# itz-sayak/C-Users-Sayakdutta-Self-Supervised-Arbitrary-Scale-Point-Cloud-Upsampling-via-SNN

Measured on AMD Instinct MI355X. Metric: upsampled query-points/sec (kNN + fn fwd + rotate + fd fwd + displace), 4x scale, M=48 T=4, higher is better.
Workload: dtype f32 (GEMMs as 3 x f16 MFMA with f32 accumulation; outer kNN f64); 1 GPU; synthetic sphere N=5000 (seed 0), B=4096 grid queries per GPU per step, M=48, T=4, fn k=[24,18,12] emb 640, fd k=32 scales [8,16,32,48] emb 768, conditioned-random weights seed 0, in-patch kNN recomputed every batch; cloud_points=5000, neighbours=48, outer_knn=f64 brute force, parallelism=query shards x1

## Files before the change

c-users-sayakdutta-self-supervised-arbitrary-scale-point-cloud-upsampling-via-snn_amd/csrc/common.h:

```cpp
#pragma once
#include <hip/hip_runtime.h>
#include <stdint.h>
#include <stdio.h>
#include <string.h>
#include "../../include/sapcu.h"

namespace sapcu {

void set_error(const char* fmt, ...);

#define SAPCU_CHECK_ARG(cond, ...)                      \
    do {                                                \
        if (!(cond)) {                                  \
            ::sapcu::set_error(__VA_ARGS__);            \
            return SAPCU_ERR_ARG;                       \
        }                                               \
    } while (0)

#define SAPCU_CHECK_HIP(expr)                                                            \
    do {                                                                                 \
        hipError_t _e = (expr);                                                          \
        if (_e != hipSuccess) {                                                          \
            ::sapcu::set_error("%s failed: %s (%s:%d)", #expr, hipGetErrorString(_e),    \
                               __FILE__, __LINE__);                                      \
// ... 343 lines not shown
    }
    __device__ __forceinline__ bool gate_open() const {
#ifdef SAPCU_LIF_EXACT_ORDER
        return sx.r <= 0.f || sy.r <= 0.f;
#else
        return s.r.x <= 0.f || s.r.y <= 0.f;
#endif
    }
    __device__ __forceinline__ f32x2 step(f32x2 x, bool first) {
#ifdef SAPCU_LIF_EXACT_ORDER
        return f32x2{neuron_step<EIF>(x.x, sx, pa), neuron_step<EIF>(x.y, sy, pb)};
#else
        f32x2 mm;
        if (first) {
            mm = x;
        } else {
            const f32x2 md = s.m * decay;
            mm = pk_fma(-md, s.r, md);
        }
        if (EIF) {
            f32x2 a = (s.m - rh) * inv_dT;
            a = f32x2{clampf(a.x, -5.0f, 5.0f), clampf(a.y, -5.0f, 5.0f)} * 1.4426950408889634074f;
            const f32x2 e = f32x2{__builtin_amdgcn_exp2f(a.x), __builtin_amdgcn_exp2f(a.y)};
            mm = pk_fma(e, dT, mm);
        }
        const f32x2 sp = soft_spike2(mm - s.th);
        s.m = pk_fma(-mm, sp, mm);
        {
            const f32x2 rn = first ? sp : pk_fma(s.r, rdecay, sp);
            s.r = f32x2{fmaxf(rn.x, SPIKE_FLOOR), fmaxf(rn.y, SPIKE_FLOOR)};
        }
        s.th = pk_fma(s.th, f32x2{0.95f, 0.95f}, pk_fma(sp, a95, thc));
        return sp;
#endif
    }
};

__device__ __forceinline__ double sqrt_cr(double d) {
    if (!(d > 0.0)) return d == 0.0 ? 0.0 : sqrt(d);
    const double s = sqrt(d);
    const double r = __fma_rn(-s, s, d);
    return __fma_rn(r, __ddiv_rn(0.5, s), s);
}

__device__ __forceinline__ float gelu_erf(float x) {
    return 0.5f * x * (1.0f + erff(x * 0.70710678118654752440f));
}
__device__ __forceinline__ float lrelu02(float x) { return x >= 0.f ? x : 0.2f * x; }
__device__ __forceinline__ unsigned float_max_key(float x) {
    const unsigned b = __float_as_uint(x);
    return (b & 0x80000000u) ? ~b : (b | 0x80000000u);
}
__device__ __forceinline__ float float_from_max_key(unsigned k) { return __uint_as_float((k & 0x80000000u) ? (k & 0x7fffffffu) : ~k); }

enum GemmEpi { EPI_BIAS = 0, EPI_LIF = 1, EPI_GELU = 2, EPI_RESID = 3, EPI_LRELU = 4, EPI_RESID_GELU = 5, EPI_LIF_ATTN = 6,
               EPI_LRELU_MAX = 7,
               EPI_LIF_MAX = 8 };

struct GemmArgs {
    const float* a;
    int64_t r;
    int k, lda;
    const float* w;
    int n;
    const float* bias;
    float* c;
    int ldc;
    int epi;
    const float* lif;
    int lif_T;
    const float* resid;
    int ldr;
    float* c2;
    const float* q;
    const float* kf;
    int ldq;
    const int2* tab;
    const _Float16* w16_hi;
    const _Float16* w16_lo;
    int* ovf;
    int a_split, c_split, c2_split;
    unsigned* max_keys;
    int max_m;
};
int launch_gemm(const GemmArgs& g, hipStream_t st);
int launch_gemm_sf16(const GemmArgs& g, hipStream_t st);
int launch_gemm_sf16_ring(const GemmArgs& g, hipStream_t st);
int launch_gemm_sf16_bt(const GemmArgs& g, hipStream_t st);
bool gemm_sf16_bt_ok(const GemmArgs& g);
int launch_gemm_split_rows(const GemmArgs& g, hipStream_t st, bool allow_bt = true);
int launch_split_weights(const float* w, int64_t count, void* hi, void* lo, int* ovf, hipStream_t st);

int launch_knn_outer(const double* cloud, int64_t n, const double* q, int64_t b, int k, int64_t* idx,
                     double* dist, float* patch, hipStream_t st);
int launch_gather_rotate(const double* cloud, int64_t n, const double* q, int64_t b, const int64_t* idx,
                         int k, const float* normals, float* patch, hipStream_t st);
int launch_displace(const double* q, const float* nrm, const float* d, int64_t b, double* out, hipStream_t st);

size_t fps_workspace_bytes(int npoint);
int launch_fps(const float* xyz, int64_t n, int npoint, int start, int64_t* out, void* ws, hipStream_t st);
int fps_failed(const void* ws, int npoint, int* flag);

}
```

c-users-sayakdutta-self-supervised-arbitrary-scale-point-cloud-upsampling-via-snn_amd/csrc/model.hip:

```cpp
#include <stdarg.h>
#include <stdlib.h>

#include <new>
#include <vector>

#include "common.h"
#include "ops.h"

namespace sapcu {

static thread_local char g_err[512] = "";

void set_error(const char* fmt, ...) {
    va_list ap;
    va_start(ap, fmt);
    vsnprintf(g_err, sizeof(g_err), fmt, ap);
    va_end(ap);
}

enum FnSlot {
    FN_STEM_W = 0, FN_STEM_B, FN_STEM_LIF,
    FN_BLK0 = 3,
    FN_FINAL_W = FN_BLK0 + 63, FN_FINAL_B, FN_FINAL_LIF,
    FN_FCOUT_W, FN_FCOUT_B,
    FN_MLP0_W, FN_MLP0_B, FN_MLP1_W, FN_MLP1_B, FN_MLP2_W, FN_MLP2_B,
    FN_HEAD_W, FN_HEAD_B, FN_LN_W, FN_LN_B,
    FN_SLOTS
};
enum FnBlkSlot {
    B_FC1_W = 0, B_FC1_B, B_SNN1,
    B_QKV_W, B_QKV_B, B_QKV_LIF,
    B_DELTA_W, B_DELTA_B, B_DELTA_LIF,
    B_DELTA2_W, B_DELTA2_B, B_DELTA2_LIF,
    B_GAMMA_W, B_GAMMA_B, B_GAMMA_LIF,
    B_GAMMA2_W, B_GAMMA2_B,
    B_OUT_W, B_OUT_B,
    B_FC2_W, B_FC2_B,
    B_SLOTS
};
static_assert(B_SLOTS == 21, "fn block slot count");
static_assert(FN_SLOTS == 81, "fn slot count");

enum FdSlot {
    FD_E0_W = 0, FD_E0_B,
    FD_FUSE_W, FD_FUSE_B, FD_SNN0,
    FD_EDGE1_W, FD_EDGE1_SHIFT, FD_SNN1,
    FD_EDGE2_W, FD_EDGE2_SHIFT, FD_SNN2,
    FD_EDGE3_W, FD_EDGE3_SHIFT, FD_SNN3,
    FD_MSC_W, FD_MSC_B,
    FD_TI_W, FD_SNNFC,
    FD_FCIN_W, FD_FCIN_B,
    FD_R0_FC0_W, FD_R0_FC0_B, FD_R0_FC4_W, FD_R0_FC4_B, FD_R0_PROJ_W, FD_R0_PROJ_B,
    FD_R1_FC0_W, FD_R1_FC0_B, FD_R1_FC4_W, FD_R1_FC4_B, FD_R1_PROJ_W, FD_R1_PROJ_B,
    FD_QKV_W, FD_QKV_B,
    FD_WO_T, FD_BO, FD_LN_W, FD_LN_B, FD_WH_T, FD_BH, FD_WD, FD_BD,
    FD_SLOTS
};
static_assert(FD_SLOTS == 42, "fd slot count");

}

struct sapcu_model {
    int kind = 0;
    int kv[3] = {0, 0, 0};
    int k = 0, nscale = 0;
    int ks[8] = {0, 0, 0, 0, 0, 0, 0, 0};
    int32_t* ks_dev = nullptr;
    int* gate_dev = nullptr;
    bool sf16 = true;
    void* w16_hi = nullptr;
    void* w16_lo = nullptr;
    void* chain_w = nullptr;
    int* ovf_dev = nullptr;
    int emb = 0, T = 0, heads = 0;
    int64_t chunk = 0;
    int64_t ws_budget = 0;
    bool opt_bt = true;
    bool opt_chain = true;
    bool opt_chain_wide = false;
    bool opt_chain_fill = true;
    bool opt_fn_maxfuse = true;
    bool opt_fn_fold_out = true;
    bool opt_fd_maxfuse = true;
    bool opt_fd_split = true;
    bool opt_fd_fused = true;
    bool opt_fd_x0 = true;
    void* fde_w = nullptr;
    int64_t fde_off[5] = {0, 0, 0, 0, 0};
    float* fde_nprm = nullptr;
    float* blob = nullptr;
    int64_t blob_floats = 0;
    int64_t fold_w[3] = {0, 0, 0}, fold_b[3] = {0, 0, 0};
    std::vector<int64_t> dir;
    const float* p(int slot) const { return blob + dir[slot]; }
};

namespace sapcu {

static inline int64_t imax(int64_t a, int64_t b) { return a > b ? a : b; }
static inline int imin(int a, int b) { return a < b ? a : b; }

static bool split_rows_gemm_on_big_tile(const GemmArgs& g, bool allow_bt) { return allow_bt && gemm_sf16_bt_ok(g); }

int launch_gemm_split_rows(const GemmArgs& g, hipStream_t st, bool allow_bt) {
    if (split_rows_gemm_on_big_tile(g, allow_bt)) return launch_gemm_sf16_bt(g, st);
    return launch_gemm_sf16_ring(g, st);
}

static void fold_affine_f64(const float* w1, const float* b1, const float* w2, const float* b2, int d, int n, float* w_fold,
                            float* b_fold) {
    std::vector<double> acc((size_t)d);
    for (int i = 0; i < n; ++i) {
        for (int k = 0; k < d; ++k) acc[k] = 0.0;
        double bs = 0.0;
        for (int j = 0; j < d; ++j) {
            const double a = (double)w2[(int64_t)i * d + j];
            const float* row = w1 + (int64_t)j * d;
            for (int k = 0; k < d; ++k) acc[k] += a * (double)row[k];
            bs += a * (double)b1[j];
        }
        for (int k = 0; k < d; ++k) w_fold[(int64_t)i * d + k] = (float)acc[k];
        b_fold[i] = (float)(bs + (double)b2[i]);
    }
}

static bool env_is(const char* name, const char* value) {
    const char* e = getenv(name);
    return e && strcmp(e, value) == 0;
}

static void read_env_switches(sapcu_model* m) {
    m->sf16 = !env_is("SAPCU_GEMM", "f32");
    m->opt_bt = !env_is("SAPCU_BT", "0");
    m->opt_chain = !env_is("SAPCU_CHAIN", "0");
    m->opt_chain_wide = env_is("SAPCU_CHAIN", "wide");
    m->opt_chain_fill = !env_is("SAPCU_CHAIN_FILL", "0");
    m->opt_fn_maxfuse = !env_is("SAPCU_FN_MAXFUSE", "0");
    m->opt_fn_fold_out = !env_is("SAPCU_FN_FOLD_OUT", "0");
    m->opt_fd_maxfuse = !env_is("SAPCU_FD_MAXFUSE", "0");
    m->opt_fd_split = !env_is("SAPCU_FD_SPLIT", "0");
    m->opt_fd_fused = !env_is("SAPCU_FD_FUSED", "0");
    m->opt_fd_x0 = !env_is("SAPCU_FD_X0", "0");
    const char* ce = getenv("SAPCU_CHUNK");
    m->chunk = ce ? atoll(ce) : 0;
    if (m->chunk < 0) m->chunk = 0;
    const char* be = getenv("SAPCU_WS_BUDGET_MB");
    m->ws_budget = (be ? atoll(be) : 20480) * (int64_t)(1 << 20);
    if (m->ws_budget < (int64_t)(64 << 20)) m->ws_budget = (int64_t)(64 << 20);
}

static void free_model(sapcu_model* m) {
    void* const owned[] = {m->w16_hi, m->w16_lo, m->chain_w, m->ovf_dev, m->blob, m->ks_dev, m->gate_dev, m->fde_w, m->fde_nprm};
    for (void* p : owned)
        if (p) (void)hipFree(p);
    delete m;
}

static int run_gemm(const sapcu_model* m, GemmArgs& g, hipStream_t st) {
    const bool have16 = m && m->sf16 && g.w >= m->blob && g.w < m->blob + m->blob_floats;
    if (have16) {
        const int64_t off = g.w - m->blob;
        g.w16_hi = (const _Float16*)m->w16_hi + off;
        g.w16_lo = (const _Float16*)m->w16_lo + off;
        g.ovf = m->ovf_dev;
        if (g.a_split) return launch_gemm_split_rows(g, st, m->opt_bt);
        if (g.k % 64 == 0) return launch_gemm_sf16(g, st);
    }
    if (g.a_split || g.c_split || g.c2_split) {
        set_error("run_gemm: split-row operands need the split-f16 kernels");
        return SAPCU_ERR_ARG;
    }
    return launch_gemm(g, st);
}

static int gemm(const sapcu_model* m, const float* a, int64_t r, int k, int lda, const float* w, int n,
                const float* bias, float* c, int ldc, int epi, hipStream_t st, const float* lif = nullptr,
                int lifT = 0, const float* resid = nullptr, int ldr = 0, int fmt = 0) {
    GemmArgs g;
    memset(&g, 0, sizeof(g));
    g.a = a; g.r = r; g.k = k; g.lda = lda; g.w = w; g.n = n; g.bias = bias; g.c = c; g.ldc = ldc;
    g.epi = epi; g.lif = lif; g.lif_T = lifT; g.resid = resid; g.ldr = ldr;
    g.a_split = fmt & 1; g.c_split = (fmt >> 1) & 1;
    return run_gemm(m, g, st);
}

#define SAPCU_TRY(expr)                 \
    do {                                \
        int _rc = (expr);               \
        if (_rc != SAPCU_OK) return _rc; \
    } while (0)

static int tap_copy(void* const* taps, int which, int64_t dst_off_bytes, const void* src, int64_t bytes,
                    hipStream_t st) {
    if (!taps || !taps[which] || bytes == 0) return SAPCU_OK;
    SAPCU_CHECK_HIP(hipMemcpyAsync((char*)taps[which] + dst_off_bytes, src, (size_t)bytes, hipMemcpyDeviceToDevice, st));
    return SAPCU_OK;
}

struct FnPlan {
    int64_t cb;
    int kk[3], kmx;
    int64_t edge_floats, edge_floats23;
};

static bool fn_block_fused(const sapcu_model* m, int l, int mp) {
    return m->sf16 && m->chain_w && m->opt_chain && fn_edge_chain_ok(128 << l, imin(m->kv[l], mp));
}

static int fn_kmax(const sapcu_model* m, int mp) {
    int kmx = 1;
    for (int l = 0; l < 3; ++l) kmx = kmx > imin(m->kv[l], mp) ? kmx : imin(m->kv[l], mp);
    return kmx;
}

static void fn_edge_floats_per_patch(const sapcu_model* m, int mp, int64_t& first, int64_t& others) {
    first = (int64_t)mp * m->emb;
    others = 0;
    for (int l = 0; l < 3; ++l) {
        if (fn_block_fused(m, l, mp)) continue;
        const int64_t e = (int64_t)mp * imin(m->kv[l], mp) * (128 << l);
        first = imax(first, e);
        others = imax(others, e);
    }
}

static int64_t fn_bytes_per_patch(const sapcu_model* m, int mp) {
    int64_t e1, e23;
    fn_edge_floats_per_patch(m, mp, e1, e23);
    int64_t idxs = 0;
    for (int l = 0; l < 3; ++l) idxs += (int64_t)mp * imin(m->kv[l], mp) * 4;
    return (e1 + 2 * e23) * 4 + idxs + (int64_t)mp * fn_kmax(m, mp) * 24 + (int64_t)mp * (64 + 192 + 512 + 1536 + 512) * 4 +
           ((int64_t)m->emb + 2048 + 1024 + 512 + 256 + 3) * 4;
}

static int64_t chunk_patches(const sapcu_model* m, int64_t b, int64_t bytes_per_patch) {
    int64_t cb = m->chunk;
    if (cb <= 0) {
        cb = m->ws_budget / (bytes_per_patch > 0 ? bytes_per_patch : 1);
        cb = cb < 64 ? 64 : (cb / 64) * 64;
    }
    if (cb > b) cb = b;
    return cb < 1 ? 1 : cb;
}

static FnPlan fn_plan(const sapcu_model* m, int64_t b, int mp) {
    FnPlan pl;
    pl.cb = chunk_patches(m, b, fn_bytes_per_patch(m, mp));
    for (int l = 0; l < 3; ++l) pl.kk[l] = imin(m->kv[l], mp);
// ... 87 lines not shown
        GemmArgs g;
        memset(&g, 0, sizeof(g));
        g.a = W.B1; g.r = R; g.k = d; g.lda = d; g.w = m->p(sb + B_DELTA2_W); g.n = d;
        g.bias = m->p(sb + B_DELTA2_B); g.c = W.B2; g.ldc = d; g.epi = EPI_LIF_ATTN;
        g.lif = m->p(sb + B_DELTA2_LIF); g.lif_T = 4; g.c2 = W.B3;
        g.q = W.QKV; g.kf = W.QKV + d; g.ldq = 3 * d; g.tab = W.tab;
        g.a_split = SP; g.c2_split = SP;
        SAPCU_TRY(launch_edge_table(idx, R, e.mp, kk, W.tab, st));
        SAPCU_TRY(run_gemm(m, g, st));
    }
    SAPCU_TRY(gemm(m, W.B3, R, d, d, m->p(sb + B_GAMMA_W), d, m->p(sb + B_GAMMA_B), W.B1, d, EPI_LIF, st, m->p(sb + B_GAMMA_LIF), 4,
                   nullptr, 0, SP | (SP << 1)));
    SAPCU_TRY(gemm(m, W.B1, R, d, d, m->p(sb + B_GAMMA2_W), d, m->p(sb + B_GAMMA2_B), W.B3, d, EPI_BIAS, st, nullptr, 0, nullptr, 0, SP));
    return launch_fn_softmax_agg(W.B3, W.B2, W.QKV + 2 * d, 3 * d, idx, e.P, e.mp, kk, d, e.sqrt_hd, W.RES, SP, st);
}

static int fn_forward(const sapcu_model* m, const float* patch, int64_t b, int mp, const int32_t* knn_in,
                      int32_t* knn_out, float* normals, void* ws, int64_t ws_bytes, void* const* taps,
                      hipStream_t st) {
    const FnPlan pl = fn_plan(m, b, mp);
    const FnWs W = fn_ws_layout(ws_align256(ws), m, pl, mp);
    if (ws_bytes < (int64_t)W.bytes + 256) {
        set_error("fn_forward: workspace %lld B < required %lld B", (long long)ws_bytes, (long long)W.bytes + 256);
        return SAPCU_ERR_WORKSPACE;
    }
    int64_t tab_off[3];
    tab_off[0] = 0;
    tab_off[1] = b * mp * pl.kk[0];
    tab_off[2] = tab_off[1] + b * mp * pl.kk[1];

    for (int64_t s = 0; s < b; s += pl.cb) {
        const int64_t cb = (b - s) < pl.cb ? (b - s) : pl.cb;
        const int64_t P = cb * mp;
        const float* pc = patch + s * mp * 3;

        if (!knn_in) SAPCU_TRY(launch_patch_knn_multi(pc, cb, (int64_t)mp * 3, mp, 3, 3, 3, pl.kk, W.idx, st));
        for (int l = 0; l < 3; ++l) {
            const int64_t cnt = P * pl.kk[l];
            if (knn_in)
                SAPCU_CHECK_HIP(hipMemcpyAsync(W.idx[l], knn_in + tab_off[l] + s * mp * pl.kk[l], cnt * 4,
                                               hipMemcpyDeviceToDevice, st));
            if (knn_out)
                SAPCU_CHECK_HIP(hipMemcpyAsync(knn_out + tab_off[l] + s * mp * pl.kk[l], W.idx[l], cnt * 4,
                                               hipMemcpyDeviceToDevice, st));
        }
        SAPCU_TRY(launch_fn_stem(pc, P, m->p(FN_STEM_W), m->p(FN_STEM_B), m->p(FN_STEM_LIF), m->T, W.feat0, st));
        SAPCU_TRY(tap_copy(taps, SAPCU_FN_TAP_STEM, s * mp * 64 * 4, W.feat0, P * 64 * 4, st));

        const float* fin = W.feat0;
        int ldin = 64;
        for (int l = 0; l < 3; ++l) {
            const int d = 128 << l;
            const int sb = FN_BLK0 + l * B_SLOTS;
            const int SP = m->sf16 ? 1 : 0;
            float* const out = W.cat + 64 * l;
            SAPCU_TRY(gemm(m, fin, P, 64, ldin, m->p(sb + B_FC1_W), d, m->p(sb + B_FC1_B), W.X, d, EPI_LIF, st,
                           m->p(sb + B_SNN1), 4, nullptr, 0, SP << 1));
            SAPCU_TRY(gemm(m, W.X, P, d, d, m->p(sb + B_QKV_W), 3 * d, m->p(sb + B_QKV_B), W.QKV, 3 * d, EPI_LIF, st,
                           m->p(sb + B_QKV_LIF), 4, nullptr, 0, SP));
            const FnEdge e{pc, P, mp, l, d, pl.kk[l], sb, SP, (float)sqrt((double)(d / m->heads)), pl.edge_floats};
            SAPCU_TRY(fn_block_fused(m, l, mp) ? fn_edge_chain_fused(m, W, e, st) : fn_edge_chain_unfused(m, W, e, st));
            if (m->opt_fn_fold_out) {
                SAPCU_TRY(gemm(m, W.RES, P, d, d, m->blob + m->fold_w[l], 64, m->blob + m->fold_b[l], out, 192, EPI_RESID, st,
                               nullptr, 0, fin, ldin, SP));
            } else {
                SAPCU_TRY(gemm(m, W.RES, P, d, d, m->p(sb + B_OUT_W), d, m->p(sb + B_OUT_B), W.X, d, EPI_BIAS, st, nullptr, 0, nullptr,
                               0, SP | (SP << 1)));
                SAPCU_TRY(gemm(m, W.X, P, d, d, m->p(sb + B_FC2_W), 64, m->p(sb + B_FC2_B), out, 192, EPI_RESID, st,
                               nullptr, 0, fin, ldin, SP));
            }
            if (taps && taps[SAPCU_FN_TAP_BLOCK1 + l]) {
                SAPCU_CHECK_HIP(hipMemcpy2DAsync((char*)taps[SAPCU_FN_TAP_BLOCK1 + l] + s * mp * 64 * 4, 64 * 4,
                                                 out, 192 * 4, 64 * 4, (size_t)P, hipMemcpyDeviceToDevice, st));
            }
            fin = out;
            ldin = 192;
        }
        if (m->sf16 && m->opt_fn_maxfuse) {
            GemmArgs g;
            memset(&g, 0, sizeof(g));
            g.a = W.cat; g.r = P; g.k = 192; g.lda = 192; g.w = m->p(FN_FINAL_W); g.n = m->emb; g.bias = m->p(FN_FINAL_B);
            g.ldc = m->emb; g.epi = EPI_LIF_MAX; g.lif = m->p(FN_FINAL_LIF); g.lif_T = m->T;
            g.max_keys = reinterpret_cast<unsigned*>(W.B1); g.max_m = mp;
            SAPCU_CHECK_HIP(hipMemsetAsync(g.max_keys, 0, (size_t)cb * m->emb * 4, st));
            SAPCU_TRY(run_gemm(m, g, st));
            SAPCU_TRY(launch_decode_max_keys(g.max_keys, cb * m->emb, W.pooled, st));
        } else {
            SAPCU_TRY(gemm(m, W.cat, P, 192, 192, m->p(FN_FINAL_W), m->emb, m->p(FN_FINAL_B), W.B1, m->emb, EPI_LIF, st,
                           m->p(FN_FINAL_LIF), m->T));
            SAPCU_TRY(launch_rowgroup_max(W.B1, cb, mp, m->emb, W.pooled, st));
        }
        SAPCU_TRY(tap_copy(taps, SAPCU_FN_TAP_POOLED, s * m->emb * 4, W.pooled, cb * m->emb * 4, st));
        SAPCU_TRY(gemm(m, W.pooled, cb, m->emb, m->emb, m->p(FN_FCOUT_W), 2048, m->p(FN_FCOUT_B), W.enc, 2048, EPI_BIAS, st));
        SAPCU_TRY(tap_copy(taps, SAPCU_FN_TAP_ENC, s * 2048 * 4, W.enc, cb * 2048 * 4, st));
        SAPCU_TRY(gemm(m, W.enc, cb, 2048, 2048, m->p(FN_MLP0_W), 1024, m->p(FN_MLP0_B), W.h1, 1024, EPI_GELU, st));
        SAPCU_TRY(gemm(m, W.h1, cb, 1024, 1024, m->p(FN_MLP1_W), 512, m->p(FN_MLP1_B), W.h2, 512, EPI_GELU, st));
        SAPCU_TRY(gemm(m, W.h2, cb, 512, 512, m->p(FN_MLP2_W), 256, m->p(FN_MLP2_B), W.h3, 256, EPI_GELU, st));
        SAPCU_TRY(launch_fn_tail(W.h3, cb, 256, m->p(FN_HEAD_W), m->p(FN_HEAD_B), m->p(FN_LN_W), m->p(FN_LN_B), W.logits,
                                 normals + s * 3, st));
        SAPCU_TRY(tap_copy(taps, SAPCU_FN_TAP_LOGITS, s * 3 * 4, W.logits, cb * 3 * 4, st));
    }
    return SAPCU_OK;
}

struct FdPlan {
    int64_t cb;
    int kmax0, kk;
    bool fused;
    bool x0path;
    bool maxfuse;
    int64_t agg_rows(int mp) const { return maxfuse ? 1 : mp; }
};

static bool fd_encoder_fused(const sapcu_model* m, int mp) {
    return m->sf16 && m->opt_fd_fused && m->fde_w && m->fde_nprm && fd_encoder_ok(mp, m->nscale, m->emb, m->T);
}

static bool fd_x0_path(const sapcu_model* m, int mp) {
    return !fd_encoder_fused(m, mp) && m->sf16 && m->opt_fd_fused && m->opt_fd_x0 && m->opt_fd_maxfuse && m->opt_fd_split && m->fde_w &&
           m->fde_nprm && fd_msc_ok(mp, m->emb, m->T);
}

static int fd_kmax0(const sapcu_model* m, int mp) {
    int kmax = 1;
    for (int i = 0; i < m->nscale; ++i) kmax = kmax > m->ks[i] ? kmax : m->ks[i];
    return imin(kmax, mp);
}

static FdPlan fd_plan(const sapcu_model* m, int64_t b, int mp) {
    FdPlan pl;
    pl.fused = fd_encoder_fused(m, mp);
    pl.x0path = fd_x0_path(m, mp);
    pl.maxfuse = m->sf16 && m->opt_fd_maxfuse;
    pl.kmax0 = fd_kmax0(m, mp);
    pl.kk = imin(m->k, mp);
    int64_t per_patch = ((int64_t)(m->T + 1) * m->emb + 256 + 3 * 128 + 3 * 64 + 192 + 64) * 4;
    if (!pl.fused) {
        const int64_t slabs = pl.x0path ? 2 : m->T;
        per_patch = (int64_t)mp * ((slabs * 960 + 960 + 1024 + 64 * (m->nscale + 1)) * 4 + (int64_t)(pl.kmax0 + 3 * pl.kk) * 4) +
                    (int64_t)m->T * pl.agg_rows(mp) * m->emb * 4 + per_patch;
    }
    pl.cb = chunk_patches(m, b, per_patch);
    return pl;
}

struct FdWs {
    int32_t* idx0;
    int32_t* idxb;
    float* E0;
    float* FUSED;
    float* SPK;
    float* F0;
    float* AB;
    float* AGG;
    float* X0;
    float *POOLED, *ENC;
    float *D1, *D2a, *D2b, *D2c, *D3a, *D3b, *D3c, *QKV, *ATT;
    size_t bytes;
};

static FdWs fd_ws_layout(void* base, const sapcu_model* m, const FdPlan& pl, int mp) {
    const int64_t cb = pl.cb, T = m->T, emb = m->emb;
    const int64_t P = pl.fused ? 0 : cb * mp;
    WsCarver c(base);
    FdWs w;
    w.idx0 = c.take<int32_t>(P * pl.kmax0);
    w.idxb = c.take<int32_t>(3 * P * pl.kk);
    w.E0 = c.take<float>(P * 64 * m->nscale);
    w.FUSED = c.take<float>(P * 64);
// ... 226 lines not shown
                    (long long)n, (long long)npoint);
    if (npoint == 0) return SAPCU_OK;
    SAPCU_CHECK_ARG(xyz && idx_out && workspace, "fps: null pointer");
    SAPCU_CHECK_ARG(((uintptr_t)workspace & 7) == 0, "fps: the workspace must be 8-byte aligned (64-bit mailboxes)");
    if (workspace_bytes < (int64_t)fps_workspace_bytes((int)npoint)) {
        set_error("fps: workspace of %lld bytes, need %lld", (long long)workspace_bytes,
                  (long long)fps_workspace_bytes((int)npoint));
        return SAPCU_ERR_WORKSPACE;
    }
    int rc = launch_fps(xyz, n, (int)npoint, (int)(n / 2), idx_out, workspace, (hipStream_t)stream);
    if (rc != SAPCU_OK) return rc;
    SAPCU_CHECK_HIP(hipStreamSynchronize((hipStream_t)stream));
    int flag = 0;
    rc = fps_failed(workspace, (int)npoint, &flag);
    if (rc != SAPCU_OK) return rc;
    if (flag) {
        set_error("fps: a workgroup of the persistent grid never arrived at the step barrier (grid not resident)");
        return SAPCU_ERR_HIP;
    }
    return SAPCU_OK;
}

int sapcu_neuron_selfloop(const float* x, int64_t rows, int channels, int steps, const float* membrane_decay,
                          const float* threshold_adapt, const float* refractory_decay, const float* threshold_base,
                          const float* delta_T, const float* theta_rh, float* spikes_out, float* membrane_out,
                          float* threshold_out, float* refractory_out, void* stream) {
    SAPCU_CHECK_ARG(x && membrane_decay && threshold_adapt && refractory_decay && threshold_base, "neuron: null pointer");
    SAPCU_CHECK_ARG((delta_T == nullptr) == (theta_rh == nullptr), "neuron: delta_T and theta_rh go together");
    SAPCU_CHECK_ARG(rows >= 0 && channels >= 1 && steps >= 1, "neuron: bad sizes");
    return launch_neuron_selfloop(x, rows, channels, steps, membrane_decay, threshold_adapt, refractory_decay,
                                  threshold_base, delta_T, theta_rh, spikes_out, membrane_out, threshold_out,
                                  refractory_out, (hipStream_t)stream);
}

int sapcu_neuron_drive(const float* x, int64_t rows, int channels, int steps, const float* membrane_decay,
                       const float* threshold_adapt, const float* refractory_decay, const float* threshold_base,
                       const float* delta_T, const float* theta_rh, int channel_pairs, float* spikes_out, float* membrane_out,
                       float* threshold_out, float* refractory_out, int* gate_open_out, void* stream) {
    SAPCU_CHECK_ARG(x && membrane_decay && threshold_adapt && refractory_decay && threshold_base, "neuron_drive: null pointer");
    SAPCU_CHECK_ARG((delta_T == nullptr) == (theta_rh == nullptr), "neuron_drive: delta_T and theta_rh go together");
    SAPCU_CHECK_ARG(rows >= 0 && channels >= 1 && steps >= 1, "neuron_drive: bad sizes");
    return launch_neuron_drive(x, rows, channels, steps, membrane_decay, threshold_adapt, refractory_decay, threshold_base, delta_T,
                               theta_rh, channel_pairs, spikes_out, membrane_out, threshold_out, refractory_out, gate_open_out,
                               (hipStream_t)stream);
}

int sapcu_patch_knn(const float* feat, int64_t b, int m, int c, int ld, int k, int32_t* idx_out, void* stream) {
    SAPCU_CHECK_ARG(feat && idx_out && b >= 0 && ld >= c, "patch_knn: bad argument");
    return launch_patch_knn(feat, b, m, c, ld, k, idx_out, (hipStream_t)stream);
}

int sapcu_l2_normalize3(const float* in, float* out, int64_t b, void* stream) {
    SAPCU_CHECK_ARG(in && out && b >= 0, "l2_normalize3: bad argument");
    return launch_l2_normalize3(in, out, b, (hipStream_t)stream);
}

static int split_into_ws(const float* w, int64_t cnt, void* w16_ws, GemmArgs& g, hipStream_t st) {
    char* base = (char*)w16_ws;
    int* ovf = (int*)(base + 4 * cnt);
    SAPCU_CHECK_HIP(hipMemsetAsync(ovf, 0, sizeof(int), st));
    SAPCU_TRY(launch_split_weights(w, cnt, base, base + 2 * cnt, ovf, st));
    g.w16_hi = (const _Float16*)base;
    g.w16_lo = (const _Float16*)(base + 2 * cnt);
    g.ovf = ovf;
    return SAPCU_OK;
}

int sapcu_gemm_f32(const float* a, int64_t r, int k, int lda, const float* w, int n, const float* bias,
                   const float* lif4, int lif_steps, float* c, int ldc, void* w16_ws, int a_split_rows, int c_split_rows,
                   void* stream) {
    SAPCU_CHECK_ARG(a && w && c && r >= 0 && n >= 1, "gemm: bad argument");
    SAPCU_CHECK_ARG(!lif4 || lif_steps >= 1, "gemm: lif_steps must be >= 1");
    SAPCU_CHECK_ARG(!(a_split_rows || c_split_rows) || w16_ws, "gemm: split rows need the split-f16 kernels (w16_ws)");
    SAPCU_CHECK_ARG(r == 0 || (k > 0 && k % 32 == 0 && lda >= k && ldc >= n), "gemm: need k %% 32 == 0, lda >= k and ldc >= n (k=%d lda=%d n=%d ldc=%d)", k, lda, n, ldc);
    SAPCU_CHECK_ARG(r == 0 || ((((uintptr_t)a | (uintptr_t)w | (uintptr_t)w16_ws) & 15) == 0 && lda % (a_split_rows ? 8 : 4) == 0),
                    "gemm: A, W and w16_ws must be 16-byte aligned, lda %% 4 == 0 (%% 8 for split rows) (lda=%d)", lda);
    GemmArgs g;
    memset(&g, 0, sizeof(g));
    g.a = a; g.r = r; g.k = k; g.lda = lda; g.w = w; g.n = n; g.bias = bias; g.c = c; g.ldc = ldc;
    g.epi = lif4 ? EPI_LIF : EPI_BIAS; g.lif = lif4; g.lif_T = lif_steps;
    g.a_split = a_split_rows ? 1 : 0; g.c_split = c_split_rows ? 1 : 0;
    if (w16_ws && (g.a_split || k % 64 == 0)) {
        SAPCU_TRY(split_into_ws(w, (int64_t)n * k, w16_ws, g, (hipStream_t)stream));
        return g.a_split ? launch_gemm_split_rows(g, (hipStream_t)stream, a_split_rows != 2) : launch_gemm_sf16(g, (hipStream_t)stream);
    }
    SAPCU_CHECK_ARG(!g.c_split, "gemm: split-row output needs k %% 64 == 0 on the f32-A path");
    return launch_gemm(g, (hipStream_t)stream);
}

int sapcu_to_split_rows(const float* in, int64_t rows, int k, int ld_in, float* out, int ld_out, void* stream) {
    SAPCU_CHECK_ARG(in && out && rows >= 0 && k >= 1 && ld_in >= k && ld_out >= k, "to_split_rows: bad argument");
    return launch_to_split_rows(in, rows, k, ld_in, out, ld_out, (hipStream_t)stream);
}

int sapcu_posenc_gemm_f32(const float* pe1, int64_t r, int d, const float* w, const float* bias, const float* lif4,
                          int lif_steps, const float* qkv, const int32_t* idx, int kk, int m_pts, float* pe_out,
                          float* attn_in_out, void* edge_table_ws, void* w16_ws, int split_rows, void* stream) {
    SAPCU_CHECK_ARG(pe1 && w && lif4 && qkv && idx && pe_out && attn_in_out && edge_table_ws && r >= 0 && d >= 32 &&
                        lif_steps >= 1 && kk >= 1 && m_pts >= 1,
                    "posenc_gemm: bad argument");
    SAPCU_CHECK_ARG(!split_rows || w16_ws, "posenc_gemm: split rows need the split-f16 kernels (w16_ws)");
    SAPCU_CHECK_ARG(d % 32 == 0, "posenc_gemm: d=%d must be a multiple of 32", d);
    SAPCU_CHECK_ARG((((uintptr_t)pe1 | (uintptr_t)w | (uintptr_t)w16_ws) & 15) == 0 && ((uintptr_t)edge_table_ws & 7) == 0,
                    "posenc_gemm: pe1, w and w16_ws must be 16-byte aligned, edge_table_ws 8-byte aligned");
    GemmArgs g;
    memset(&g, 0, sizeof(g));
    g.a = pe1; g.r = r; g.k = d; g.lda = d; g.w = w; g.n = d; g.bias = bias; g.c = pe_out; g.ldc = d;
    g.epi = EPI_LIF_ATTN; g.lif = lif4; g.lif_T = lif_steps; g.c2 = attn_in_out;
    g.q = qkv; g.kf = qkv + d; g.ldq = 3 * d; g.tab = (const int2*)edge_table_ws;
    SAPCU_TRY(launch_edge_table(idx, r, m_pts, kk, (int2*)edge_table_ws, (hipStream_t)stream));
    if (w16_ws && (split_rows || d % 64 == 0)) {
        SAPCU_TRY(split_into_ws(w, (int64_t)d * d, w16_ws, g, (hipStream_t)stream));
        if (split_rows) {
            g.a_split = 1;
            g.c2_split = 1;
            return launch_gemm_split_rows(g, (hipStream_t)stream, split_rows != 2);
        }
        return launch_gemm_sf16(g, (hipStream_t)stream);
    }
    return launch_gemm(g, (hipStream_t)stream);
}

struct ChainWs {
    int2* tab;
    float4* pd;
    char* split[3];
    _Float16* packed[3];
    size_t bytes;
};

static ChainWs chain_ws_layout(void* base, int64_t points, int d, int kk) {
    WsCarver c(base);
    ChainWs w;
    w.tab = c.take<int2>(points * kk);
    w.pd = c.take<float4>(points * kk);
    for (int q = 0; q < 3; ++q) {
        w.split[q] = c.take<char>((int64_t)d * d * 4 + 16);
        w.packed[q] = c.take<_Float16>((int64_t)d * d * 2);
    }
    w.bytes = c.bytes();
    return w;
}

int64_t sapcu_fn_edge_chain_workspace_bytes(int64_t points, int d, int kk) {
    if (points < 0 || !fn_edge_chain_ok(d, kk)) {
        set_error("fn_edge_chain_workspace_bytes: unsupported shape (d=%d kk=%d)", d, kk);
        return SAPCU_ERR_ARG;
    }
    return (int64_t)chain_ws_layout(nullptr, points, d, kk).bytes + 256;
}

int sapcu_fn_edge_chain_f32(const float* patch, const int32_t* idx, int64_t points, int m_pts, int d, int kk,
                            const float* qkv, const float* w_delta, const float* b_delta, const float* lif_delta,
                            const float* w1, const float* b1, const float* lif1, const float* w2, const float* b2,
                            const float* lif2, const float* w3, const float* b3, int heads, int lif_steps,
                            float* res_out, void* workspace, int64_t workspace_bytes, void* stream) {
    SAPCU_CHECK_ARG(patch && idx && qkv && w_delta && b_delta && lif_delta && w1 && b1 && lif1 && w2 && b2 && lif2 && w3 && b3 &&
                        res_out && workspace, "fn_edge_chain: null pointer");
    SAPCU_CHECK_ARG(fn_edge_chain_ok(d, kk), "fn_edge_chain: unsupported shape (d=%d kk=%d)", d, kk);
    SAPCU_CHECK_ARG(points >= 0 && m_pts >= kk && heads >= 1 && d % heads == 0 && lif_steps >= 1, "fn_edge_chain: bad sizes");
    const int64_t need = sapcu_fn_edge_chain_workspace_bytes(points, d, kk);
    if (workspace_bytes < need) {
        set_error("fn_edge_chain: workspace %lld B < required %lld B", (long long)workspace_bytes, (long long)need);
        return SAPCU_ERR_WORKSPACE;
    }
    hipStream_t st = (hipStream_t)stream;
    const ChainWs W = chain_ws_layout(ws_align256(workspace), points, d, kk);
// ... 249 lines not shown
```

Baseline: 128,600 query-points/s.

## Add short-K split-f16 GEMM kernel with direct per-patch max output

```diff
diff --git a/c-users-sayakdutta-self-supervised-arbitrary-scale-point-cloud-upsampling-via-snn_amd/csrc/common.h b/c-users-sayakdutta-self-supervised-arbitrary-scale-point-cloud-upsampling-via-snn_amd/csrc/common.h
--- a/c-users-sayakdutta-self-supervised-arbitrary-scale-point-cloud-upsampling-via-snn_amd/csrc/common.h
+++ b/c-users-sayakdutta-self-supervised-arbitrary-scale-point-cloud-upsampling-via-snn_amd/csrc/common.h
@@ -449,12 +449,15 @@
     int a_split, c_split, c2_split;
     unsigned* max_keys;
     int max_m;
+    float* max_out;
 };
 int launch_gemm(const GemmArgs& g, hipStream_t st);
 int launch_gemm_sf16(const GemmArgs& g, hipStream_t st);
 int launch_gemm_sf16_ring(const GemmArgs& g, hipStream_t st);
 int launch_gemm_sf16_bt(const GemmArgs& g, hipStream_t st);
 bool gemm_sf16_bt_ok(const GemmArgs& g);
+bool gemm_shortk_ok(const GemmArgs& g);
+int launch_gemm_shortk(const GemmArgs& g, hipStream_t st);
 int launch_gemm_split_rows(const GemmArgs& g, hipStream_t st, bool allow_bt = true);
 int launch_split_weights(const float* w, int64_t count, void* hi, void* lo, int* ovf, hipStream_t st);
 
diff --git a/c-users-sayakdutta-self-supervised-arbitrary-scale-point-cloud-upsampling-via-snn_amd/csrc/gemm_shortk.hip b/c-users-sayakdutta-self-supervised-arbitrary-scale-point-cloud-upsampling-via-snn_amd/csrc/gemm_shortk.hip
--- /dev/null
+++ b/c-users-sayakdutta-self-supervised-arbitrary-scale-point-cloud-upsampling-via-snn_amd/csrc/gemm_shortk.hip
@@ -0,0 +1,177 @@
+#include "common.h"
+#include "gemm_epi.h"
+
+namespace sapcu {
+
+typedef _Float16 sk_half8 __attribute__((ext_vector_type(8)));
+
+constexpr int SK_MAX_WAVES = 8;
+
+__device__ __forceinline__ int sk_chunk_offset(int row, int chunk, int k) {
+    return row * (k * 2) + (((chunk & ~7) | ((chunk & 7) ^ ((row >> 1) & 7))) * 16);
+}
+
+template <int EPI, int RT>
+__global__ __launch_bounds__(SK_MAX_WAVES * 64, 4) void gemm_shortk_kernel(const GemmArgs g) {
+    extern __shared__ __attribute__((aligned(16))) unsigned char sk_smem[];
+    constexpr int RG = 32 * RT;
+    const int tid = threadIdx.x;
+    const int lane = tid & 63, wave = tid >> 6;
+    const int nw = blockDim.x >> 6;
+    const int r32 = lane & 31, h = lane >> 5;
+    const int K = g.k;
+    const int plane_bytes = RG * K * 2;
+    const int64_t row0 = (int64_t)blockIdx.x * RG;
+
+    {
+        const int cpr = K >> 3;
+        const int total = RG * cpr;
+        float amax = 0.f;
+        for (int c = tid; c < total; c += blockDim.x) {
+            const int row = c / cpr, ch = c - row * cpr;
+            int64_t grow = row0 + row;
+            if (grow >= g.r) grow = g.r - 1;
+            const float* ap = g.a + grow * g.lda + ch * 8;
+            const float4 x0 = ld4(ap), x1 = ld4(ap + 4);
+            const float xs[8] = {x0.x, x0.y, x0.z, x0.w, x1.x, x1.y, x1.z, x1.w};
+            sk_half8 hi, lo;
+#pragma unroll
+            for (int i = 0; i < 8; ++i) {
+                const _Float16 hh = (_Float16)xs[i];
+                hi[i] = hh;
+                lo[i] = (_Float16)(xs[i] - (float)hh);
+                amax = fmaxf(amax, fabsf(xs[i]));
+            }
+            const int off = sk_chunk_offset(row, ch, K);
+            *reinterpret_cast<sk_half8*>(sk_smem + off) = hi;
+            *reinterpret_cast<sk_half8*>(sk_smem + plane_bytes + off) = lo;
+        }
+        if (amax > 65504.0f && g.ovf) atomicAdd(g.ovf, 1);
+    }
+    __syncthreads();
+
+    const int nct = (g.n + 31) >> 5;
+    const int nk = K >> 6;
+    for (int ct = wave; ct < nct; ct += nw) {
+        const int col = ct * 32 + r32;
+        const bool col_ok = col < g.n;
+        const int cc = col_ok ? col : g.n - 1;
+        const _Float16* wp[2] = {g.w16_hi + (int64_t)cc * K + h * 8, g.w16_lo + (int64_t)cc * K + h * 8};
+        f32x16 acc[RT];
+#pragma unroll
+        for (int rt = 0; rt < RT; ++rt)
+#pragma unroll
+            for (int e = 0; e < 16; ++e) acc[rt][e] = 0.f;
+
+        sk_half8 wa[2][2], wb[2][2];
+        auto load_w = [&](sk_half8 (&w)[2][2], int k32) {
+#pragma unroll
+            for (int p = 0; p < 2; ++p)
+#pragma unroll
+                for (int t = 0; t < 2; ++t) w[p][t] = *reinterpret_cast<const sk_half8*>(wp[p] + k32 * 32 + t * 16);
+        };
+        auto step = [&](const sk_half8 (&w)[2][2], int k32) {
+            auto product = [&](int a_plane, int w_plane) {
+#pragma unroll
+                for (int t = 0; t < 2; ++t)
+#pragma unroll
+                    for (int rt = 0; rt < RT; ++rt) {
+                        const sk_half8 a = *reinterpret_cast<const sk_half8*>(
+                            sk_smem + a_plane * plane_bytes + sk_chunk_offset(rt * 32 + r32, (2 * k32 + t) * 2 + h, K));
+                        acc[rt] = __builtin_amdgcn_mfma_f32_32x32x16_f16(a, w[w_plane][t], acc[rt], 0, 0, 0);
+                    }
+            };
+            product(1, 0);
+            product(0, 1);
+            product(0, 0);
+        };
+        load_w(wa, 0);
+        for (int kt = 0; kt < nk; ++kt) {
+            load_w(wb, 2 * kt + 1);
+            step(wa, 2 * kt);
+            if (kt + 1 < nk) load_w(wa, 2 * kt + 2);
+            step(wb, 2 * kt + 1);
+        }
+
+        const float bias = g.bias ? g.bias[cc] : 0.f;
+        const NeuronP np = load_lif(g.lif, g.n, cc);
+        const int off_f32 = 4 * h * g.ldc + col;
+        const int off_hi = 8 * h * g.ldc + split_hi_index(g.ldc, col), off_lo = 8 * h * g.ldc + split_lo_index(g.ldc, col);
+        float pmax[2] = {-INFINITY, -INFINITY};
+#pragma unroll
+        for (int rt = 0; rt < RT; ++rt) {
+#pragma unroll
+            for (int half = 0; half < 2; ++half) {
+                const int64_t grow = row0 + rt * 32 + half * 16;
+                if (grow >= g.r) continue;
+                __builtin_amdgcn_sched_barrier(0);
+                float v[8];
+#pragma unroll
+                for (int e = 0; e < 8; ++e) v[e] = __fadd_rn(__fmul_rn(acc[rt][half * 8 + e], 0.0625f), bias);
+                lif_selfloop_n<8>(v, np, g.lif_T);
+                if (EPI == EPI_LIF_MAX) {
+                    float best = v[0];
+#pragma unroll
+                    for (int e = 1; e < 8; ++e) best = fmaxf(best, v[e]);
+                    const int pi = (rt * 2 + half) >= 3 ? 1 : 0;
+                    pmax[pi] = fmaxf(pmax[pi], best);
+                } else {
+                    const int left = (g.r - grow) < 16 ? (int)(g.r - grow) : 16;
+#pragma unroll
+                    for (int e = 0; e < 8; ++e) {
+                        const int lr = 8 * (e >> 2) + (e & 3);
+                        float* rowp = g.c + (grow + lr) * g.ldc;
+                        if (!col_ok || lr + 4 * h >= left) continue;
+                        if (g.c_split) {
+                            _Float16* rp = reinterpret_cast<_Float16*>(rowp);
+                            const _Float16 hi = (_Float16)v[e];
+                            rp[off_hi] = hi;
+                            rp[off_lo] = (_Float16)(v[e] - (float)hi);
+                        } else {
+                            rowp[off_f32] = v[e];
+                        }
+                    }
+                }
+            }
+        }
+        if (EPI == EPI_LIF_MAX) {
+            pmax[0] = fmaxf(pmax[0], __shfl_xor(pmax[0], 32));
+            pmax[1] = fmaxf(pmax[1], __shfl_xor(pmax[1], 32));
+            float* op = g.max_out + (int64_t)blockIdx.x * 2 * g.ldc;
+            const int left = (g.r - row0) < RG ? (int)(g.r - row0) : RG;
+            if (col_ok && h * 48 < left) op[h * g.ldc + col] = h ? pmax[1] : pmax[0];
+        }
+    }
+}
+
+bool gemm_shortk_ok(const GemmArgs& g) {
+    if (g.a_split || !g.w16_hi || !g.w16_lo || !g.lif || g.lif_T < 1) return false;
+    if (g.k < 64 || g.k > 192 || g.k % 64 != 0) return false;
+    if (g.r >= ((int64_t)1 << 31) * 32) return false;
+    if (g.epi == EPI_LIF) return true;
+    return g.epi == EPI_LIF_MAX && g.max_out && g.max_m == 48 && g.r % 48 == 0;
+}
+
+template <int EPI, int RT>
+static int launch_shortk_t(const GemmArgs& g, hipStream_t st) {
+    static DeviceOnce lds_once;
+    constexpr int RG = 32 * RT;
+    SAPCU_SET_MAX_LDS(lds_once, (&gemm_shortk_kernel<EPI, RT>), RG * 192 * 4);
+    const int nct = (g.n + 31) / 32;
+    const int nw = nct < SK_MAX_WAVES ? nct : SK_MAX_WAVES;
+    const int64_t groups = (g.r + RG - 1) / RG;
+    hipLaunchKernelGGL((gemm_shortk_kernel<EPI, RT>), dim3((unsigned)groups), dim3(nw * 64), (size_t)RG * g.k * 4, st, g);
+    SAPCU_CHECK_LAUNCH();
+    return SAPCU_OK;
+}
+
+int launch_gemm_shortk(const GemmArgs& g, hipStream_t st) {
+    if (g.r == 0 || g.n == 0) return SAPCU_OK;
+    SAPCU_CHECK_ARG(gemm_shortk_ok(g), "gemm_shortk: shape or epilogue not served (k=%d epi=%d)", g.k, g.epi);
+    SAPCU_CHECK_ARG(g.lda % 4 == 0 && ((uintptr_t)g.a & 15) == 0 && ((uintptr_t)g.w16_hi & 15) == 0 && ((uintptr_t)g.w16_lo & 15) == 0,
+                    "gemm_shortk: operands must be 16-byte aligned (lda=%d)", g.lda);
+    if (g.epi == EPI_LIF_MAX) return launch_shortk_t<EPI_LIF_MAX, 3>(g, st);
+    return launch_shortk_t<EPI_LIF, 2>(g, st);
+}
+
+}
diff --git a/c-users-sayakdutta-self-supervised-arbitrary-scale-point-cloud-upsampling-via-snn_amd/csrc/model.hip b/c-users-sayakdutta-self-supervised-arbitrary-scale-point-cloud-upsampling-via-snn_amd/csrc/model.hip
--- a/c-users-sayakdutta-self-supervised-arbitrary-scale-point-cloud-upsampling-via-snn_amd/csrc/model.hip
+++ b/c-users-sayakdutta-self-supervised-arbitrary-scale-point-cloud-upsampling-via-snn_amd/csrc/model.hip
@@ -79,6 +79,7 @@
     bool opt_chain = true;
     bool opt_chain_wide = false;
     bool opt_chain_fill = true;
+    bool opt_shortk = true;
     bool opt_fn_maxfuse = true;
     bool opt_fn_fold_out = true;
     bool opt_fd_maxfuse = true;
@@ -135,6 +136,7 @@
     m->opt_chain = !env_is("SAPCU_CHAIN", "0");
     m->opt_chain_wide = env_is("SAPCU_CHAIN", "wide");
     m->opt_chain_fill = !env_is("SAPCU_CHAIN_FILL", "0");
+    m->opt_shortk = !env_is("SAPCU_SHORTK", "0");
     m->opt_fn_maxfuse = !env_is("SAPCU_FN_MAXFUSE", "0");
     m->opt_fn_fold_out = !env_is("SAPCU_FN_FOLD_OUT", "0");
     m->opt_fd_maxfuse = !env_is("SAPCU_FD_MAXFUSE", "0");
@@ -164,6 +166,11 @@
         g.w16_lo = (const _Float16*)m->w16_lo + off;
         g.ovf = m->ovf_dev;
         if (g.a_split) return launch_gemm_split_rows(g, st, m->opt_bt);
+        if (m->opt_shortk && gemm_shortk_ok(g)) return launch_gemm_shortk(g, st);
+        if (g.max_out) {
+            set_error("run_gemm: a direct max output needs the short-K kernel");
+            return SAPCU_ERR_ARG;
+        }
         if (g.k % 64 == 0) return launch_gemm_sf16(g, st);
     }
     if (g.a_split || g.c_split || g.c2_split) {
@@ -417,9 +424,11 @@
             g.a = W.cat; g.r = P; g.k = 192; g.lda = 192; g.w = m->p(FN_FINAL_W); g.n = m->emb; g.bias = m->p(FN_FINAL_B);
             g.ldc = m->emb; g.epi = EPI_LIF_MAX; g.lif = m->p(FN_FINAL_LIF); g.lif_T = m->T;
             g.max_keys = reinterpret_cast<unsigned*>(W.B1); g.max_m = mp;
-            SAPCU_CHECK_HIP(hipMemsetAsync(g.max_keys, 0, (size_t)cb * m->emb * 4, st));
+            const bool direct = m->opt_shortk && mp == 48;
+            if (direct) g.max_out = W.pooled;
+            else SAPCU_CHECK_HIP(hipMemsetAsync(g.max_keys, 0, (size_t)cb * m->emb * 4, st));
             SAPCU_TRY(run_gemm(m, g, st));
-            SAPCU_TRY(launch_decode_max_keys(g.max_keys, cb * m->emb, W.pooled, st));
+            if (!direct) SAPCU_TRY(launch_decode_max_keys(g.max_keys, cb * m->emb, W.pooled, st));
         } else {
             SAPCU_TRY(gemm(m, W.cat, P, 192, 192, m->p(FN_FINAL_W), m->emb, m->p(FN_FINAL_B), W.B1, m->emb, EPI_LIF, st,
                            m->p(FN_FINAL_LIF), m->T));
@@ -812,7 +821,9 @@
     g.a_split = a_split_rows ? 1 : 0; g.c_split = c_split_rows ? 1 : 0;
     if (w16_ws && (g.a_split || k % 64 == 0)) {
         SAPCU_TRY(split_into_ws(w, (int64_t)n * k, w16_ws, g, (hipStream_t)stream));
-        return g.a_split ? launch_gemm_split_rows(g, (hipStream_t)stream, a_split_rows != 2) : launch_gemm_sf16(g, (hipStream_t)stream);
+        if (g.a_split) return launch_gemm_split_rows(g, (hipStream_t)stream, a_split_rows != 2);
+        if (!env_is("SAPCU_SHORTK", "0") && gemm_shortk_ok(g)) return launch_gemm_shortk(g, (hipStream_t)stream);
+        return launch_gemm_sf16(g, (hipStream_t)stream);
     }
     SAPCU_CHECK_ARG(!g.c_split, "gemm: split-row output needs k %% 64 == 0 on the f32-A path");
     return launch_gemm(g, (hipStream_t)stream);
```

Result: faster. 130,700 query-points/s, median of 6 (+1.7%).
